# abdur75648/AI-Camera

Measured on AMD Instinct MI355X. Metric: end-to-end frames/sec @1280x720, 30 persons/frame, higher is better.
Workload: dtype f16

## Files before the change

ai-camera_amd/csrc/kernels_conv_block.hip:

```cpp
#include "conv_common.hpp"

namespace aic {

struct BlockArgs {
    const void* x; void* y;
    const void* w1; const float* b1;
    const void* w2; const float* b2;
    const void* zero;
    int x_cs, x_coff, y_cs, y_coff, H, n_img, ipb;
    const int* n_dev;
};

__global__ __launch_bounds__(512) void conv3x3_c64_block_kernel(const BlockArgs a) {
    constexpr int PW = 34, ROWB = PW * 128, IN_ROWS = 20, MID_ROWS = 16;
    constexpr int MID_OFF = IN_ROWS * ROWB, DUMMY_OFF = MID_OFF + MID_ROWS * ROWB, BIAS_OFF = DUMMY_OFF + 1024;
    extern __shared__ __attribute__((aligned(16))) char smem[];

    const int t = threadIdx.x, lane = t & 63, wv = __builtin_amdgcn_readfirstlane(t >> 6), r = lane & 15, q = lane >> 4;
    const int grp = wv >> 2, cx = wv & 1, ch = (wv >> 1) & 1;
    const half_t* __restrict__ xg = reinterpret_cast<const half_t*>(a.x);
    const half_t* zero = reinterpret_cast<const half_t*>(a.zero);
    const half_t* __restrict__ wg = reinterpret_cast<const half_t*>(grp ? a.w2 : a.w1);
    const float* bg = grp ? a.b2 : a.b1;

    half8 wreg[18][2];
#pragma unroll
    for (int j = 0; j < 2; ++j) {
        const half_t* wr = wg + (size_t)(32 * ch + perm_row<2>(j, r)) * 576 + 8 * q;
#pragma unroll
        for (int s2 = 0; s2 < 18; ++s2) wreg[s2][j] = *reinterpret_cast<const half8*>(wr + 32 * s2);
    }
#pragma unroll
    for (int s2 = 0; s2 < 18; ++s2) asm volatile("" :: "v"(wreg[s2][0]), "v"(wreg[s2][1]));
    float* bias_l = reinterpret_cast<float*>(smem + BIAS_OFF) + ((grp * 2 + ch) * 4 + q) * 8;
    if (cx == 0 && r == 0) {
#pragma unroll
        for (int j = 0; j < 2; ++j)
#pragma unroll
            for (int e = 0; e < 4; ++e) bias_l[4 * j + e] = bg[32 * ch + perm_ch<2>(j, q, e)];
    }
    for (int o = t * 16; o < MID_ROWS * ROWB; o += 512 * 16) *reinterpret_cast<uint4*>(smem + MID_OFF + o) = make_uint4(0u, 0u, 0u, 0u);

    const int gpi = a.H / 4 + 1;
    const int n_live = a.n_dev ? min(a.n_img, a.n_dev[0]) : a.n_img;
    const int ipb = a.n_dev ? (n_live + (int)gridDim.x - 1) / (int)gridDim.x : a.ipb;
    const int img0 = blockIdx.x * ipb;
    const int n_loc = max(0, min(ipb, n_live - img0));
    const int S_tot = gpi * n_loc;

    int doff[3];
#pragma unroll
    for (int p = 0; p < 3; ++p) {
        const int sl = (p * 8 + wv) * 64 + lane;
        const int rr = sl / 272, rem = sl - rr * 272;
        const int px = rem >> 3, c = (rem & 7) ^ (px & 7);
        doff[p] = (p * 8 + wv < 17 && (unsigned)(px - 1) < 32u) ? (rr * 32 + (px - 1)) * a.x_cs + a.x_coff + c * 8 : -1;
    }
    auto issue = [&](int g) {
        int gs = g % 5; if (gs < 0) gs += 5;
        const int jl = g >= 0 ? g / gpi : 0, gy = g - jl * gpi;
        const bool real = g >= 0 && jl < n_loc && gy < gpi - 1;
        const half_t* gbase = xg + ((size_t)(img0 + jl) * a.H + gy * 4) * 32 * a.x_cs;
#pragma unroll
        for (int p = 0; p < 3; ++p) {
            const int j = p * 8 + wv;
            const half_t* src = (real && doff[p] >= 0) ? gbase + doff[p] : zero;
            asm volatile("" : "+v"(src));
            char* dst = j < 17 ? smem + gs * 4 * ROWB + j * 1024 : smem + DUMMY_OFF;
            __builtin_amdgcn_global_load_lds((gptr_t)src, (lptr_t)dst, 16, 0, 0);
        }
    };

    int xk[3];
#pragma unroll
    for (int kw = 0; kw < 3; ++kw) {
        const int px = cx * 16 + r + kw;
        xk[kw] = (px * 8 + (q ^ (px & 7))) * 16;
    }
    const int px1 = cx * 16 + r + 1;
    const int mid_w = (px1 * 8 + ((4 * ch + q) ^ (px1 & 7))) * 16;

    half_t* yg = reinterpret_cast<half_t*>(a.y);
    const unsigned yl0 = (unsigned)((((cx * 16 + r) * a.y_cs) + a.y_coff + 32 * ch + 8 * q) * 2);
    const unsigned rl0 = (unsigned)((((cx * 16 + r) * a.x_cs) + a.x_coff + 32 * ch + 8 * q) * 2);
    const unsigned ystep = (unsigned)(32 * a.y_cs * 2), rstep = (unsigned)(32 * a.x_cs * 2);

    floatx4 acc[4][2];
    half8 rv[4];
    half8 xf[6];
    int rowb[6];
    auto xread = [&xf, &xk, &rowb](auto g, auto ir) {
        constexpr int gg = decltype(g)::value, ii = decltype(ir)::value, kw = gg >> 1;
        const int ad = ((gg & 1) ? (xk[kw] ^ 64) : xk[kw]) + rowb[ii];
        asm volatile("ds_read_b128 %0, %1" : "=v"(xf[ii]) : "v"(ad));
    };
    auto xwait = [&xf](auto n, auto ir) {
        asm volatile("s_waitcnt lgkmcnt(%1)" : "+v"(xf[decltype(ir)::value]) : "n"(decltype(n)::value));
    };
    auto kfirst = [&]() {
        static_for<6>([&](auto ir) { xread(std::integral_constant<int, 0>{}, ir); });
#pragma unroll
        for (int i = 0; i < 4; ++i)
#pragma unroll
            for (int j = 0; j < 2; ++j) acc[i][j] = *reinterpret_cast<const floatx4*>(bias_l + 4 * j);
    };
    auto kpart = [&](auto part) {
        static_for<3>([&](auto gi) {
            constexpr int g = 3 * decltype(part)::value + decltype(gi)::value, kw = g >> 1, cc = g & 1;
            static_for<6>([&](auto ir_c) {
                constexpr int ir = decltype(ir_c)::value;
                xwait(std::integral_constant<int, (g == 5 ? 5 - ir : 5)>{}, ir_c);
#pragma unroll
                for (int kh = 0; kh < 3; ++kh) {
                    const int i = ir - kh;
                    if (i < 0 || i > 3) continue;
#pragma unroll
                    for (int j = 0; j < 2; ++j)
                        acc[i][j] = __builtin_amdgcn_mfma_f32_16x16x32_f16(wreg[(kh * 3 + kw) * 2 + cc][j], xf[ir], acc[i][j], 0, 0, 0);
                }
                if constexpr (g + 1 < 6) xread(std::integral_constant<int, g + 1>{}, ir_c);
                __builtin_amdgcn_sched_barrier(0);
            });
        });
    };
    using P0 = std::integral_constant<int, 0>;
    using P1 = std::integral_constant<int, 1>;

    auto rows1 = [&](int s) {
#pragma unroll
        for (int ir = 0; ir < 6; ++ir) {
            const int v = 4 * s - 1 + ir;
            int gsl = (v >> 2) % 5; if (gsl < 0) gsl += 5;
            rowb[ir] = (gsl * 4 + (v & 3)) * ROWB;
        }
    };
    auto store_mid = [&](int s) {
#pragma unroll
        for (int i = 0; i < 4; ++i) {
            float v[8];
#pragma unroll
            for (int e = 0; e < 8; ++e) v[e] = act_fast<2>(acc[i][e >> 2][e & 3]);
            const half8 o = {(half_t)v[0], (half_t)v[1], (half_t)v[2], (half_t)v[3], (half_t)v[4], (half_t)v[5], (half_t)v[6], (half_t)v[7]};
            const int ad = MID_OFF + ((4 * s + i) & 15) * ROWB + mid_w;
            asm volatile("ds_write_b128 %0, %1" :: "v"(ad), "v"(o) : "memory");
        }
    };
    auto zero_mid = [&](int s) {
        const half8 o = {0, 0, 0, 0, 0, 0, 0, 0};
#pragma unroll
        for (int i = 0; i < 4; ++i) {
            const int ad = MID_OFF + ((4 * s + i) & 15) * ROWB + mid_w;
            asm volatile("ds_write_b128 %0, %1" :: "v"(ad), "v"(o) : "memory");
        }
    };
    auto load_res = [&](size_t pix0) {
        const char* rb = reinterpret_cast<const char*>(xg) + pix0 * a.x_cs * 2;
        unsigned rl = rl0;
        asm volatile("" : "+v"(rl));
#pragma unroll
        for (int i = 0; i < 4; ++i)
            asm volatile("global_load_dwordx4 %0, %1, %2" : "=v"(rv[i]) : "v"(rl + i * rstep), "s"(rb) : "memory");
    };
    auto rows2 = [&](int tt) {
#pragma unroll
        for (int ir = 0; ir < 6; ++ir) rowb[ir] = MID_OFF + ((4 * tt - 1 + ir) & 15) * ROWB;
    };
    auto store_out = [&](size_t pix0) {
        asm volatile("s_waitcnt vmcnt(3)" : "+v"(rv[0]), "+v"(rv[1]), "+v"(rv[2]), "+v"(rv[3]) :: "memory");
        char* yb = reinterpret_cast<char*>(yg) + pix0 * a.y_cs * 2;
        unsigned yl = yl0;
        asm volatile("" : "+v"(yl));
#pragma unroll
        for (int i = 0; i < 4; ++i) {
            float v[8];
#pragma unroll
            for (int e = 0; e < 8; ++e) v[e] = act_fast<2>(acc[i][e >> 2][e & 3] + (float)rv[i][e]);
            const half8 o = {(half_t)v[0], (half_t)v[1], (half_t)v[2], (half_t)v[3], (half_t)v[4], (half_t)v[5], (half_t)v[6], (half_t)v[7]};
            *reinterpret_cast<half8*>(yb + (size_t)(yl + i * ystep)) = o;
        }
    };

    issue(-1); issue(0); issue(1); issue(2);
    asm volatile("s_waitcnt lgkmcnt(0)" ::: "memory");
    if (grp == 0) {
        for (int s = 0; s < S_tot + 2; ++s) {
            wait_vmcnt<3>();
            __builtin_amdgcn_s_barrier();
            issue(s + 3);
            const bool live = s < S_tot, act1 = live && s % gpi < gpi - 1;
            if (act1) {
                rows1(s);
                kfirst();
                kpart(P0{});
            }
            __builtin_amdgcn_s_barrier();
            if (live) {
                if (act1) {
                    kpart(P1{});
                    store_mid(s);
                } else zero_mid(s);
                asm volatile("s_waitcnt lgkmcnt(0)" ::: "memory");
            }
        }
        __builtin_amdgcn_s_barrier();
    } else {
        wait_vmcnt<3>();
        __builtin_amdgcn_s_barrier();
        bool prev = false;
        for (int s = 0; s < S_tot + 2; ++s) {
            __builtin_amdgcn_s_barrier();
            const int tt = s - 2;
            const bool act2 = tt >= 0 && tt < S_tot && (tt % gpi) < gpi - 1;
            const int jl = act2 ? tt / gpi : 0, gy = act2 ? tt % gpi : 0;
            const size_t pix0 = ((size_t)(img0 + jl) * a.H + gy * 4) * 32;
            if (act2) load_res(pix0);
            issue(s + 3);
            if (act2) {
                rows2(tt);
                kfirst();
                kpart(P0{});
            }
            if (act2 && prev) wait_vmcnt<11>();
            else if (act2 || prev) wait_vmcnt<7>();
            else wait_vmcnt<3>();
            __builtin_amdgcn_s_barrier();
            if (act2) {
                kpart(P1{});
                store_out(pix0);
            }
            prev = act2;
        }
    }
    wait_vmcnt<0>();
}

void launch_c64_block(const ConvArgs& c1, const ConvArgs& c2, int ipb, hipStream_t s) {
    BlockArgs a{};
    a.x = c1.x, a.y = c2.y, a.w1 = c1.w, a.b1 = c1.bias, a.w2 = c2.w, a.b2 = c2.bias, a.zero = c1.zero;
    a.x_cs = c1.x_cs, a.x_coff = c1.x_coff, a.y_cs = c2.y_cs, a.y_coff = c2.y_coff, a.H = c1.H;
    a.n_img = c1.M / (c1.H * c1.W);
    a.n_dev = c1.n_dev;
    a.ipb = ipb;
    constexpr size_t lds = (size_t)(20 + 16) * 34 * 128 + 1024 + 512;
    set_lds_limit(conv3x3_c64_block_kernel, lds);
    hipLaunchKernelGGL(conv3x3_c64_block_kernel, dim3((a.n_img + a.ipb - 1) / a.ipb), dim3(512), lds, s, a);
    KCHECK();
}

}
```

Measured before the change: 12100.

## Strength-reduce ring-buffer addressing and use immediate LDS offsets in fused conv block

The fused two-conv residual block kernel drops its per-step div/mod address math. The input ring slot order is permuted so one conv1 step's rows sit within a 16-bit ds_read offset of a base, and the loop is unrolled by five so those offsets become immediates. The fetch pointer, residual pointer and mid-ring row advance incrementally. It also uses inline-asm MFMAs with manual s_nop hazard padding, s_setprio around the second compute phase, and a plain ReLU via v_max for the mid activation. The aim is less scalar/VALU address overhead in a tight MFMA pipeline. The price is fragile hand-managed hazards and more code from unrolling.

```diff
diff --git a/ai-camera_amd/csrc/kernels_conv_block.hip b/ai-camera_amd/csrc/kernels_conv_block.hip
--- a/ai-camera_amd/csrc/kernels_conv_block.hip
+++ b/ai-camera_amd/csrc/kernels_conv_block.hip
@@ -11,9 +11,37 @@
     const int* n_dev;
 };
 
+namespace blk {
+constexpr int PW = 34, ROWB = PW * 128, IN_ROWS = 20, MID_ROWS = 16;
+constexpr int MID_OFF = IN_ROWS * ROWB, DUMMY_OFF = MID_OFF + MID_ROWS * ROWB, BIAS_OFF = DUMMY_OFF + 1024, LDS = BIAS_OFF + 512;
+static_assert((MID_ROWS - 1) * ROWB < 65536, "a ring row's offset from its wave's base fits ds_read's 16-bit immediate");
+__host__ __device__ constexpr int in_slot(int g) { return 2 * g % 5; }
+__host__ __device__ constexpr int in_row(int u, int ir) {
+    return ir == 0 ? 4 * in_slot((u + 4) % 5) + 3 : ir <= 4 ? 4 * in_slot(u) + ir - 1 : 4 * in_slot((u + 1) % 5);
+}
+__host__ __device__ constexpr int row_base(int u) {
+    int m = in_row(u, 0);
+    for (int ir = 1; ir < 6; ++ir) m = in_row(u, ir) < m ? in_row(u, ir) : m;
+    return m;
+}
+constexpr bool rows_in_reach() {
+    for (int u = 0; u < 5; ++u)
+        for (int ir = 0; ir < 6; ++ir)
+            if (in_row(u, ir) - row_base(u) > 15) return false;
+    return true;
+}
+static_assert(rows_in_reach(), "every row of a conv1 step within 15 rows of the step's base");
+}
+
+template <int OFF> __device__ __forceinline__ void ds_read16(half8& x, int base) {
+    asm volatile("ds_read_b128 %0, %1 offset:%2" : "=v"(x) : "v"(base), "n"(OFF));
+}
+template <int OFF> __device__ __forceinline__ void ds_write16(int base, const half8& x) {
+    asm volatile("ds_write_b128 %0, %1 offset:%2" :: "v"(base), "v"(x), "n"(OFF) : "memory");
+}
+
 __global__ __launch_bounds__(512) void conv3x3_c64_block_kernel(const BlockArgs a) {
-    constexpr int PW = 34, ROWB = PW * 128, IN_ROWS = 20, MID_ROWS = 16;
-    constexpr int MID_OFF = IN_ROWS * ROWB, DUMMY_OFF = MID_OFF + MID_ROWS * ROWB, BIAS_OFF = DUMMY_OFF + 1024;
+    using namespace blk;
     extern __shared__ __attribute__((aligned(16))) char smem[];
 
     const int t = threadIdx.x, lane = t & 63, wv = __builtin_amdgcn_readfirstlane(t >> 6), r = lane & 15, q = lane >> 4;
@@ -32,12 +60,12 @@
     }
 #pragma unroll
     for (int s2 = 0; s2 < 18; ++s2) asm volatile("" :: "v"(wreg[s2][0]), "v"(wreg[s2][1]));
-    float* bias_l = reinterpret_cast<float*>(smem + BIAS_OFF) + ((grp * 2 + ch) * 4 + q) * 8;
+    const int bias_l = BIAS_OFF + ((grp * 2 + ch) * 4 + q) * 32;
     if (cx == 0 && r == 0) {
 #pragma unroll
         for (int j = 0; j < 2; ++j)
 #pragma unroll
-            for (int e = 0; e < 4; ++e) bias_l[4 * j + e] = bg[32 * ch + perm_ch<2>(j, q, e)];
+            for (int e = 0; e < 4; ++e) reinterpret_cast<float*>(smem + bias_l)[4 * j + e] = bg[32 * ch + perm_ch<2>(j, q, e)];
     }
     for (int o = t * 16; o < MID_ROWS * ROWB; o += 512 * 16) *reinterpret_cast<uint4*>(smem + MID_OFF + o) = make_uint4(0u, 0u, 0u, 0u);
 
@@ -56,55 +84,50 @@
         const int px = rem >> 3, c = (rem & 7) ^ (px & 7);
         doff[p] = (p * 8 + wv < 17 && (unsigned)(px - 1) < 32u) ? (rr * 32 + (px - 1)) * a.x_cs + a.x_coff + c * 8 : -1;
     }
-    auto issue = [&](int g) {
-        int gs = g % 5; if (gs < 0) gs += 5;
-        const int jl = g >= 0 ? g / gpi : 0, gy = g - jl * gpi;
-        const bool real = g >= 0 && jl < n_loc && gy < gpi - 1;
-        const half_t* gbase = xg + ((size_t)(img0 + jl) * a.H + gy * 4) * 32 * a.x_cs;
-#pragma unroll
-        for (int p = 0; p < 3; ++p) {
+    const half_t* f_src = xg + (size_t)img0 * a.H * 32 * a.x_cs;
+    int f_gy = -1, f_jl = 0, f_slot = in_slot(4);
+    const size_t gstride = (size_t)128 * a.x_cs;
+    auto issue = [&]() {
+        const bool real = f_gy >= 0 && f_gy < gpi - 1 && f_jl < n_loc;
+        auto dma = [&](auto pc, const half_t* src) {
+            constexpr int p = decltype(pc)::value;
             const int j = p * 8 + wv;
-            const half_t* src = (real && doff[p] >= 0) ? gbase + doff[p] : zero;
             asm volatile("" : "+v"(src));
-            char* dst = j < 17 ? smem + gs * 4 * ROWB + j * 1024 : smem + DUMMY_OFF;
+            char* dst = j < 17 ? smem + f_slot * 4 * ROWB + j * 1024 : smem + DUMMY_OFF;
             __builtin_amdgcn_global_load_lds((gptr_t)src, (lptr_t)dst, 16, 0, 0);
-        }
-    };
-
-    int xk[3];
+        };
+        if (real) static_for<3>([&](auto pc) { dma(pc, doff[pc] >= 0 ? f_src + doff[pc] : zero); });
+        else static_for<3>([&](auto pc) { dma(pc, zero); });
+        if (real) f_src += gstride;
+        f_slot = f_slot >= 3 ? f_slot - 3 : f_slot + 2;
+        if (++f_gy == gpi) f_gy = 0, ++f_jl;
+    };
+
+    int lp[6];
 #pragma unroll
     for (int kw = 0; kw < 3; ++kw) {
         const int px = cx * 16 + r + kw;
-        xk[kw] = (px * 8 + (q ^ (px & 7))) * 16;
+        lp[2 * kw] = (px * 8 + (q ^ (px & 7))) * 16;
+        lp[2 * kw + 1] = lp[2 * kw] ^ 64;
     }
     const int px1 = cx * 16 + r + 1;
     const int mid_w = (px1 * 8 + ((4 * ch + q) ^ (px1 & 7))) * 16;
-
-    half_t* yg = reinterpret_cast<half_t*>(a.y);
-    const unsigned yl0 = (unsigned)((((cx * 16 + r) * a.y_cs) + a.y_coff + 32 * ch + 8 * q) * 2);
-    const unsigned rl0 = (unsigned)((((cx * 16 + r) * a.x_cs) + a.x_coff + 32 * ch + 8 * q) * 2);
-    const unsigned ystep = (unsigned)(32 * a.y_cs * 2), rstep = (unsigned)(32 * a.x_cs * 2);
 
     floatx4 acc[4][2];
     half8 rv[4];
     half8 xf[6];
-    int rowb[6];
-    auto xread = [&xf, &xk, &rowb](auto g, auto ir) {
-        constexpr int gg = decltype(g)::value, ii = decltype(ir)::value, kw = gg >> 1;
-        const int ad = ((gg & 1) ? (xk[kw] ^ 64) : xk[kw]) + rowb[ii];
-        asm volatile("ds_read_b128 %0, %1" : "=v"(xf[ii]) : "v"(ad));
-    };
     auto xwait = [&xf](auto n, auto ir) {
         asm volatile("s_waitcnt lgkmcnt(%1)" : "+v"(xf[decltype(ir)::value]) : "n"(decltype(n)::value));
     };
-    auto kfirst = [&]() {
-        static_for<6>([&](auto ir) { xread(std::integral_constant<int, 0>{}, ir); });
-#pragma unroll
-        for (int i = 0; i < 4; ++i)
-#pragma unroll
-            for (int j = 0; j < 2; ++j) acc[i][j] = *reinterpret_cast<const floatx4*>(bias_l + 4 * j);
-    };
-    auto kpart = [&](auto part) {
+    auto kfirst = [&](auto rd) {
+#pragma unroll
+        for (int i = 0; i < 4; ++i) {
+            asm volatile("ds_read_b128 %0, %1" : "=v"(acc[i][0]) : "v"(bias_l));
+            asm volatile("ds_read_b128 %0, %1 offset:16" : "=v"(acc[i][1]) : "v"(bias_l));
+        }
+        static_for<6>([&](auto ir) { rd(std::integral_constant<int, 0>{}, ir); });
+    };
+    auto kpart = [&](auto part, auto rd) {
         static_for<3>([&](auto gi) {
             constexpr int g = 3 * decltype(part)::value + decltype(gi)::value, kw = g >> 1, cc = g & 1;
             static_for<6>([&](auto ir_c) {
@@ -116,119 +139,145 @@
                     if (i < 0 || i > 3) continue;
 #pragma unroll
                     for (int j = 0; j < 2; ++j)
-                        acc[i][j] = __builtin_amdgcn_mfma_f32_16x16x32_f16(wreg[(kh * 3 + kw) * 2 + cc][j], xf[ir], acc[i][j], 0, 0, 0);
-                }
-                if constexpr (g + 1 < 6) xread(std::integral_constant<int, g + 1>{}, ir_c);
+                        asm volatile("v_mfma_f32_16x16x32_f16 %0, %1, %2, %0" : "+v"(acc[i][j]) : "v"(wreg[(kh * 3 + kw) * 2 + cc][j]), "v"(xf[ir]));
+                }
+                if constexpr (g + 1 < 6) rd(std::integral_constant<int, g + 1>{}, ir_c);
                 __builtin_amdgcn_sched_barrier(0);
             });
         });
     };
+    auto acc_ready = []() { asm volatile("s_nop 15\n\ts_nop 15" ::: "memory"); };
     using P0 = std::integral_constant<int, 0>;
     using P1 = std::integral_constant<int, 1>;
 
-    auto rows1 = [&](int s) {
-#pragma unroll
-        for (int ir = 0; ir < 6; ++ir) {
-            const int v = 4 * s - 1 + ir;
-            int gsl = (v >> 2) % 5; if (gsl < 0) gsl += 5;
-            rowb[ir] = (gsl * 4 + (v & 3)) * ROWB;
-        }
-    };
-    auto store_mid = [&](int s) {
-#pragma unroll
-        for (int i = 0; i < 4; ++i) {
-            float v[8];
-#pragma unroll
-            for (int e = 0; e < 8; ++e) v[e] = act_fast<2>(acc[i][e >> 2][e & 3]);
-            const half8 o = {(half_t)v[0], (half_t)v[1], (half_t)v[2], (half_t)v[3], (half_t)v[4], (half_t)v[5], (half_t)v[6], (half_t)v[7]};
-            const int ad = MID_OFF + ((4 * s + i) & 15) * ROWB + mid_w;
-            asm volatile("ds_write_b128 %0, %1" :: "v"(ad), "v"(o) : "memory");
-        }
-    };
-    auto zero_mid = [&](int s) {
-        const half8 o = {0, 0, 0, 0, 0, 0, 0, 0};
-#pragma unroll
-        for (int i = 0; i < 4; ++i) {
-            const int ad = MID_OFF + ((4 * s + i) & 15) * ROWB + mid_w;
-            asm volatile("ds_write_b128 %0, %1" :: "v"(ad), "v"(o) : "memory");
-        }
-    };
-    auto load_res = [&](size_t pix0) {
-        const char* rb = reinterpret_cast<const char*>(xg) + pix0 * a.x_cs * 2;
-        unsigned rl = rl0;
-        asm volatile("" : "+v"(rl));
-#pragma unroll
-        for (int i = 0; i < 4; ++i)
-            asm volatile("global_load_dwordx4 %0, %1, %2" : "=v"(rv[i]) : "v"(rl + i * rstep), "s"(rb) : "memory");
-    };
-    auto rows2 = [&](int tt) {
-#pragma unroll
-        for (int ir = 0; ir < 6; ++ir) rowb[ir] = MID_OFF + ((4 * tt - 1 + ir) & 15) * ROWB;
-    };
-    auto store_out = [&](size_t pix0) {
-        asm volatile("s_waitcnt vmcnt(3)" : "+v"(rv[0]), "+v"(rv[1]), "+v"(rv[2]), "+v"(rv[3]) :: "memory");
-        char* yb = reinterpret_cast<char*>(yg) + pix0 * a.y_cs * 2;
-        unsigned yl = yl0;
-        asm volatile("" : "+v"(yl));
-#pragma unroll
-        for (int i = 0; i < 4; ++i) {
-            float v[8];
-#pragma unroll
-            for (int e = 0; e < 8; ++e) v[e] = act_fast<2>(acc[i][e >> 2][e & 3] + (float)rv[i][e]);
-            const half8 o = {(half_t)v[0], (half_t)v[1], (half_t)v[2], (half_t)v[3], (half_t)v[4], (half_t)v[5], (half_t)v[6], (half_t)v[7]};
-            *reinterpret_cast<half8*>(yb + (size_t)(yl + i * ystep)) = o;
-        }
-    };
-
-    issue(-1); issue(0); issue(1); issue(2);
+    issue(); issue(); issue(); issue();
     asm volatile("s_waitcnt lgkmcnt(0)" ::: "memory");
+    const int n_steps = S_tot + 2;
     if (grp == 0) {
-        for (int s = 0; s < S_tot + 2; ++s) {
-            wait_vmcnt<3>();
-            __builtin_amdgcn_s_barrier();
-            issue(s + 3);
-            const bool live = s < S_tot, act1 = live && s % gpi < gpi - 1;
-            if (act1) {
-                rows1(s);
-                kfirst();
-                kpart(P0{});
-            }
-            __builtin_amdgcn_s_barrier();
-            if (live) {
+        int xb[6];
+#pragma unroll
+        for (int g = 0; g < 6; ++g) xb[g] = lp[g] + row_base(0) * ROWB;
+        int gy = 0;
+        for (int s0 = 0; s0 < n_steps; s0 += 5) {
+            static_for<5>([&](auto uc) {
+                constexpr int u = decltype(uc)::value;
+                const int s = s0 + u;
+                if (s >= n_steps) return;
+                if constexpr (row_base(u) != row_base((u + 4) % 5)) {
+#pragma unroll
+                    for (int g = 0; g < 6; ++g) {
+                        xb[g] += (row_base(u) - row_base((u + 4) % 5)) * ROWB;
+                        asm volatile("" : "+v"(xb[g]));
+                    }
+                }
+                auto rd = [&](auto gc, auto irc) {
+                    constexpr int g = decltype(gc)::value, ir = decltype(irc)::value;
+                    ds_read16<(in_row(u, ir) - row_base(u)) * ROWB>(xf[ir], xb[g]);
+                };
+                wait_vmcnt<3>();
+                __builtin_amdgcn_s_barrier();
+                issue();
+                const bool live = s < S_tot, act1 = live && gy < gpi - 1;
                 if (act1) {
-                    kpart(P1{});
-                    store_mid(s);
-                } else zero_mid(s);
-                asm volatile("s_waitcnt lgkmcnt(0)" ::: "memory");
-            }
+                    kfirst(rd);
+                    kpart(P0{}, rd);
+                }
+                __builtin_amdgcn_s_barrier();
+                if (live) {
+                    const int mb = MID_OFF + (s & 3) * 4 * ROWB + mid_w;
+                    if (act1) {
+                        __builtin_amdgcn_s_setprio(1);
+                        kpart(P1{}, rd);
+                        acc_ready();
+                        static_for<4>([&](auto ic) {
+                            constexpr int i = decltype(ic)::value;
+                            float v[8];
+#pragma unroll
+                            for (int e = 0; e < 8; ++e)
+                                asm("v_max_f32 %0, 0, %1" : "=v"(v[e]) : "v"(acc[i][e >> 2][e & 3]));
+                            const half8 o = {(half_t)v[0], (half_t)v[1], (half_t)v[2], (half_t)v[3], (half_t)v[4], (half_t)v[5], (half_t)v[6], (half_t)v[7]};
+                            ds_write16<i * ROWB>(mb, o);
+                        });
+                    } else {
+                        const half8 o = {0, 0, 0, 0, 0, 0, 0, 0};
+                        static_for<4>([&](auto ic) { ds_write16<decltype(ic)::value * ROWB>(mb, o); });
+                    }
+                    asm volatile("s_waitcnt lgkmcnt(0)" ::: "memory");
+                    __builtin_amdgcn_s_setprio(0);
+                }
+                if (++gy == gpi) gy = 0;
+            });
         }
         __builtin_amdgcn_s_barrier();
     } else {
+        int xk[3];
+#pragma unroll
+        for (int kw = 0; kw < 3; ++kw) xk[kw] = lp[2 * kw];
+        half_t* yg = reinterpret_cast<half_t*>(a.y);
+        const unsigned yl0 = (unsigned)((((cx * 16 + r) * a.y_cs) + a.y_coff + 32 * ch + 8 * q) * 2);
+        const unsigned rl0 = (unsigned)((((cx * 16 + r) * a.x_cs) + a.x_coff + 32 * ch + 8 * q) * 2);
+        const unsigned ystep = (unsigned)(32 * a.y_cs * 2), rstep = (unsigned)(32 * a.x_cs * 2);
+        size_t pix0 = (size_t)img0 * a.H * 32;
+        int gy = -2;
+        int mrow = MID_OFF + 8 * ROWB;
         wait_vmcnt<3>();
         __builtin_amdgcn_s_barrier();
         bool prev = false;
-        for (int s = 0; s < S_tot + 2; ++s) {
+        for (int s = 0; s < n_steps; ++s) {
             __builtin_amdgcn_s_barrier();
-            const int tt = s - 2;
-            const bool act2 = tt >= 0 && tt < S_tot && (tt % gpi) < gpi - 1;
-            const int jl = act2 ? tt / gpi : 0, gy = act2 ? tt % gpi : 0;
-            const size_t pix0 = ((size_t)(img0 + jl) * a.H + gy * 4) * 32;
-            if (act2) load_res(pix0);
-            issue(s + 3);
+            const bool act2 = gy >= 0 && s - 2 < S_tot && gy < gpi - 1;
+            const char* rb = reinterpret_cast<const char*>(xg) + pix0 * a.x_cs * 2;
             if (act2) {
-                rows2(tt);
-                kfirst();
-                kpart(P0{});
+                unsigned rl = rl0;
+                asm volatile("" : "+v"(rl));
+#pragma unroll
+                for (int i = 0; i < 4; ++i)
+                    asm volatile("global_load_dwordx4 %0, %1, %2" : "=v"(rv[i]) : "v"(rl + i * rstep), "s"(rb) : "memory");
+            }
+            issue();
+            int rowb[6];
+            rowb[0] = mrow == MID_OFF ? MID_OFF + 15 * ROWB : mrow - ROWB;
+#pragma unroll
+            for (int ir = 1; ir < 5; ++ir) rowb[ir] = mrow + (ir - 1) * ROWB;
+            rowb[5] = mrow == MID_OFF + 12 * ROWB ? MID_OFF : mrow + 4 * ROWB;
+            auto rd = [&](auto gc, auto irc) {
+                constexpr int g = decltype(gc)::value, ir = decltype(irc)::value;
+                ds_read16<0>(xf[ir], ((g & 1) ? (xk[g >> 1] ^ 64) : xk[g >> 1]) + rowb[ir]);
+            };
+            if (act2) {
+                static_for<6>([&](auto ir) { rd(std::integral_constant<int, 0>{}, ir); });
+#pragma unroll
+                for (int i = 0; i < 4; ++i)
+#pragma unroll
+                    for (int j = 0; j < 2; ++j) acc[i][j] = *reinterpret_cast<const floatx4*>(smem + bias_l + 16 * j);
+                kpart(P0{}, rd);
             }
             if (act2 && prev) wait_vmcnt<11>();
             else if (act2 || prev) wait_vmcnt<7>();
             else wait_vmcnt<3>();
             __builtin_amdgcn_s_barrier();
             if (act2) {
-                kpart(P1{});
-                store_out(pix0);
+                __builtin_amdgcn_s_setprio(1);
+                kpart(P1{}, rd);
+                acc_ready();
+                asm volatile("s_waitcnt vmcnt(3)" : "+v"(rv[0]), "+v"(rv[1]), "+v"(rv[2]), "+v"(rv[3]) :: "memory");
+                char* yb = reinterpret_cast<char*>(yg) + pix0 * a.y_cs * 2;
+                unsigned yl = yl0;
+                asm volatile("" : "+v"(yl));
+#pragma unroll
+                for (int i = 0; i < 4; ++i) {
+                    float v[8];
+#pragma unroll
+                    for (int e = 0; e < 8; ++e) v[e] = act_fast<2>(acc[i][e >> 2][e & 3] + (float)rv[i][e]);
+                    const half8 o = {(half_t)v[0], (half_t)v[1], (half_t)v[2], (half_t)v[3], (half_t)v[4], (half_t)v[5], (half_t)v[6], (half_t)v[7]};
+                    *reinterpret_cast<half8*>(yb + (size_t)(yl + i * ystep)) = o;
+                }
+                pix0 += 128;
+                __builtin_amdgcn_s_setprio(0);
             }
             prev = act2;
+            if (++gy == gpi) gy = 0;
+            mrow = mrow == MID_OFF + 12 * ROWB ? MID_OFF : mrow + 4 * ROWB;
         }
     }
     wait_vmcnt<0>();
@@ -241,7 +290,7 @@
     a.n_img = c1.M / (c1.H * c1.W);
     a.n_dev = c1.n_dev;
     a.ipb = ipb;
-    constexpr size_t lds = (size_t)(20 + 16) * 34 * 128 + 1024 + 512;
+    constexpr size_t lds = blk::LDS;
     set_lds_limit(conv3x3_c64_block_kernel, lds);
     hipLaunchKernelGGL(conv3x3_c64_block_kernel, dim3((a.n_img + a.ipb - 1) / a.ipb), dim3(512), lds, s, a);
     KCHECK();
```

New measurement: 12270 (median of 6 runs). +1.4%, better.
